# Xinglab/abPOA

Measured on AMD Instinct MI355X. Metric: read-sets/sec (consensus bit-exact) + DP Gcells/sec (roofline.dp_gcells_per_s), higher is better.
Workload: dtype int16

## Files before the change

abpoa_amd/csrc/engine.cpp:

```cpp
#include <hip/hip_runtime.h>
#include <stdio.h>
#include <stdlib.h>
#include <string.h>
#include <stdarg.h>
#include <limits.h>
#include <mutex>
#include <vector>
#include <algorithm>
#include "engine_options.h"
#include "batch_stream.h"
#include "dir_plane.h"

namespace abpoa_hip {

static char g_err[512] = ""; static std::mutex g_err_mu;
static thread_local char g_err_copy[512] = "";
static thread_local char tl_err[512] = "";
void set_err(const char *fmt, ...) {
    va_list ap; va_start(ap, fmt); vsnprintf(tl_err, sizeof(tl_err), fmt, ap); va_end(ap);
    std::lock_guard<std::mutex> lk(g_err_mu);
    memcpy(g_err, tl_err, sizeof(g_err));
}
const char *thread_last_error() { return tl_err; }
void clear_thread_error() { tl_err[0] = 0; }
// ... 184 lines not shown
                                b.lds.fr_cols > 0 &&
                                d.qlen <= b.lds.q_cap && !(dbg_ & 64);
            const bool dir_a = dir && fast_a && (dir_wide || !takes_wide_band(b.lds, d.w));
            d.plane_cap = dir_a ? (first_pass ? dir_est_cells_[todo[t]] : dir_full_cells_[todo[t]]) : (first_pass ? est_cells_[todo[t]] : full_cells_[todo[t]]);
            d.plane_off = plane_bytes; plane_bytes += (int64_t)align_up((size_t)d.plane_cap * (d.bits / 8) + 64 * 8 * 4);
            pass[t] = d;
        }
        if ((rc = planes_.reserve((size_t)plane_bytes))) return rc;
        memcpy(hi + o_desc_, pass.data(), sizeof(AlnDesc) * pass.size());
        b.o1 = sc->gap_open1; b.e1 = sc->gap_ext1; b.o2 = sc->gap_open2; b.e2 = sc->gap_ext2;
        b.align_mode = sc->align_mode; b.gap_mode = sc->gap_mode; b.wb = sc->wb; b.zdrop = sc->zdrop; b.ret_cigar = sc->ret_cigar; b.rev_cigar = sc->rev_cigar;
        b.want_trace = trace ? 1 : 0; b.fresh_band = fresh ? 1 : 0;
        b.dir_mode = dir ? (dir_wide ? 2 : 1) : 0; b.row_sdist = di + o_sdist_; b.row_pd = (const uint32_t *)(di + o_pd_);
        b.want_lr = (trace || (flags_ & BS_WANT_BAND_STATE)) ? 1 : 0;
        b.dbg = opt_int("ABPOA_HIP_DBG", 0);
        b.mat = (const int32_t *)(di + o_mat_); b.aln = (const AlnDesc *)(di + o_desc_); b.out = (AlnOut *)(dout + o_rec_);
        b.query = di + o_query_; b.row_base = di + o_base_; b.row_node_id = (const int32_t *)(di + o_nid_); b.row_remain = (const int32_t *)(di + o_rem_);
        b.row_active = di + o_act_; b.pred_off = (const int32_t *)(di + o_poff_); b.pred_row = (const int32_t *)(di + o_pred_);
        b.out_off = (const int32_t *)(di + o_ooff_); b.out_row = (const int32_t *)(di + o_out_);
        b.left = (int32_t *)(dout + o_left_); b.right = (int32_t *)(dout + o_right_);
        b.dp_beg_sn = (int32_t *)(dout + o_bsn_); b.dp_end_sn = (int32_t *)(dout + o_esn_); b.row_cell_off = (int64_t *)(dout + o_coff_);
        b.row_max_i = (int32_t *)(dout + o_rmi_); b.planes = planes_.dev; b.cigar = (uint64_t *)(dout + o_cig_);

        HIP_TRY(hipEventRecord(ev_[0], stream_), ABPOA_HIP_ELAUNCH);
        HIP_TRY(hipMemcpyAsync(di, hi, first_pass ? in_bytes_ : o_mat_, hipMemcpyHostToDevice, stream_), ABPOA_HIP_ELAUNCH);
        if (banded && !fresh) {
            if (first_pass) {
                saved_lr.assign((const int32_t *)(ho + o_left_), (const int32_t *)(ho + o_left_) + lr_words);
                HIP_TRY(hipMemcpyAsync(dout + o_left_, ho + o_left_, lr_words * 4, hipMemcpyHostToDevice, stream_), ABPOA_HIP_ELAUNCH);
            } else for (int i : todo) {
// ... 245 lines not shown
```

abpoa_amd/csrc/engine_options.cpp:

```cpp
#include "engine_options.h"
#include <atomic>
#include <cstdlib>
#include <cstring>
#include <mutex>
#include <string>

namespace abpoa_hip {
namespace {

struct Row { const char *name, *help; };
const Row kTable[] = {
    {"ABPOA_GPU_DEVICES", "P  device ordinals abpoa_hip_msa_batch spreads its batches over: all | 0,1,... (default: the device of abpoa_hip_init)"},
    {"ABPOA_GPU_BATCHES_PER_DEVICE", "P  batches dealt per device queue [2]"},
    {"ABPOA_HIP_STRICT", "P  1: a call that would hand any read-set to the host driver fails with ABPOA_HIP_ESTRICT"},
    {"ABPOA_HIP_VERBOSE", "P  per-pass timings, residency and fallback reasons on stderr"},
    {"ABPOA_HIP_HOSTGRAPH", "T  1: the host driver for every job"},
    {"ABPOA_HIP_NO_DEVICE_STRAND", "T  1: -s jobs on the host driver"},
    {"ABPOA_HIP_NO_DEVICE_LOCAL", "T  1: local-mode jobs on the host driver"},
    {"ABPOA_HIP_NO_DEVICE_GENERAL", "T  1: general-kernel jobs on the host driver"},
    {"ABPOA_HIP_DEVICE_GENERAL", "T  1: the general kernel for every device-resident job"},
    {"ABPOA_HIP_LOCKSTEP", "T  1: one launch per phase and round also where the all-rounds kernel would run"},
    {"ABPOA_HIP_LATE_TAIL", "T  1: the helpers of the all-rounds kernel's backtrack start after the row loop, not under it"},
    {"ABPOA_HIP_NODIR", "T  1: score-record arenas instead of direction words"},
    {"ABPOA_HIP_DIR_WIDE", "T  1 / 0: direction words for wide-band alignments always / never (default: by residency and memory)"},
    {"ABPOA_HIP_NOFAST", "T  1: no fast row loops (general kernel)"},
    {"ABPOA_HIP_NOWIDE", "T  1: no wide row loop"},
    {"ABPOA_HIP_NOXL", "T  1: no long-read form of the wide row loop"},
    {"ABPOA_HIP_LOCAL_TEAM", "T  1 / 0: the four-wavefront local row loop always / never"},
    {"ABPOA_HIP_WIDE_LO", "T  smallest band half-width that takes the wide loop [40]"},
    {"ABPOA_HIP_RING_ROWS", "T  depth of the wide loop's score ring (4 | 8 | 16)"},
    {"ABPOA_HIP_EXTRA_ROUTE_MIN", "T  ragged sets with fewer extra columns keep the narrow loop"},
    {"ABPOA_HIP_NO_RAGGED_SPLIT", "T  1: read-sets with ragged read ends stay in the batch of the uniform ones (no all-rounds kernel for such a job)"},
    {"ABPOA_HIP_RAGGED_CONCURRENT", "T  1: the ragged batch of a mixed job runs on a second queue of the device beside the uniform batch (measured: see LOG.md)"},
    {"ABPOA_HIP_PASS_SETS", "T  read-sets per pass of the device-resident driver"},
    {"ABPOA_HIP_FIRST_PASS", "T  start the node-slot ladder (3x, 4.5x, 6x, 4096x) at its second / third / fourth pass: 1 / 2 / 3 (profiling runs of one step)"},
    {"ABPOA_HIP_NO_PASS_HINT", "T  1: always start the ladder at 3x"},
    {"ABPOA_HIP_GROUPS", "T  read-set groups of the host driver"},
    {"ABPOA_HIP_ARENA_PCT", "T  arena estimate in percent (overflow-retry tests)"},
    {"ABPOA_HIP_BT_BYTES", "T  LDS window of the tail kernel in bytes"},
    {"ABPOA_HIP_BT_WC", "T  columns per row of the tail's column-slice windows"},
    {"ABPOA_HIP_ORDER_LDS", "T  0: the row-order walk with global tables"},
    {"ABPOA_HIP_ORDER_CAP", "T  node capacity of the row-order walk's LDS tables"},
    {"ABPOA_HIP_DBG", "D  bit mask handed to the kernels (DevBatch.dbg: 64 no fast loops, 128 keep counters, 1024 one wavefront per backtrack, 2048 the compiler's tight loop, ...)"},
    {"ABPOA_HIP_DEVSYNC", "D  1: compare device graph / row order / MSA with the host's after every read"},
    {"ABPOA_HIP_DEVICE_AUDIT", "D  1: every pool of a device queue must sit on that queue's device"},
    {"ABPOA_HIP_CIGAR_DIGEST", "D  1: fold every graph cigar into a per-set digest on the device"},
    {"ABPOA_HIP_DIRTRACE", "D  1: keep direction words and scores (word-level tests)"},
    {"ABPOA_HIP_IMBAL", "D  1: per-round mean / slowest alignment"},
    {"ABPOA_HIP_WIDE_COUNTERS", "D  path census of the wide loop (diagnostic build)"},
    {"ABPOA_HIP_ROW_CENSUS", "D  row census of the narrow loop (diagnostic build)"},
    {"ABPOA_HIP_ORDER_PROF", "D  in-kernel clock of the row-order walk (diagnostic build)"},
};
constexpr int N = (int)(sizeof(kTable) / sizeof(kTable[0]));

struct Snap { bool set[N]; std::string val[N]; };
std::mutex g_mu;
bool g_over_on[N]; std::string g_over[N];
std::atomic<const Snap *> g_snap{nullptr};
// ... 43 lines not shown
```

abpoa_amd/csrc/msa_device.cpp:

```cpp
#include <algorithm>
#include <atomic>
#include <chrono>
#include <limits.h>
#include <mutex>
#include <stdio.h>
#include <stdlib.h>
#include <string.h>
#include <thread>
#include <vector>
#include <hip/hip_runtime.h>
#include "engine_options.h"
#include "batch_stream.h"
#include "msa_device.h"
#include "poa_device.h"
#include "poa_graph.h"
#include "dir_plane.h"
#include "msa_batch.h"
#include "msa_device_debug.h"
#include "msa_device_plan.h"

namespace abpoa_hip {

namespace {
#define HIP_OK(expr, code) do { hipError_t e_ = (expr); if (e_ != hipSuccess) { \
// ... 283 lines not shown
    b.lds.narrow_off = (!mixed && b.lds.wide_on >= 1 && w_min >= b.lds.wide_w_lo && w_top <= b.lds.wide_w_hi) ? 1 : 0;
    return 0;
}

int fill_dev_batch(Job &J, bool *want_general) {
    const DevicePlan &pl = J.pl; Cache &C = *J.C; const Layout &L = J.L; const abpoa_hip_scoring_t *sc = &pl.sc; const PoaDev &p = J.p; DevBatch &b = J.b, &b_rc = J.b_rc;
    uint8_t *di = C.in.dev, *dr = C.rows.dev; const bool gen_io = pl.gen_io(); int rc;
    memset(&b, 0, sizeof(b));
    b.n = J.n_sets; b.m = sc->m;
    if ((rc = final_lds_plan(J, b))) return rc;
    if (!pl.local && !pl.general && (b.lds.fr_cols == 0 || pl.max_qlen > b.lds.q_cap)) { *want_general = true; set_err("band too wide for the fast row loop"); return ABPOA_HIP_EINVAL; }
    b.o1 = sc->gap_open1; b.e1 = sc->gap_ext1; b.o2 = sc->gap_open2; b.e2 = sc->gap_ext2;
    b.align_mode = sc->align_mode; b.gap_mode = sc->gap_mode; b.wb = sc->wb; b.zdrop = sc->zdrop; b.ret_cigar = 1; b.rev_cigar = 0;
    b.want_trace = 0; b.fresh_band = 1; b.want_lr = 0;
    b.dbg = opt_int("ABPOA_HIP_DBG", 0);
    b.mat = (const int32_t *)(di + L.o_mat); b.aln = p.aln; b.out = p.out;
    b.dir_mode = pl.dir ? (pl.dir_wide ? 2 : 1) : 0; b.row_sdist = p.row_sdist; b.row_pd = p.row_pd;
    b.query = p.reads; b.row_base = p.row_base; b.row_node_id = p.row_node_id; b.row_remain = p.row_remain; b.row_active = p.row_base;
    b.pred_off = p.pred_off; b.pred_row = p.pred_row; b.out_off = p.pred_off; b.out_row = p.pred_row;
    b.left = p.scratch; b.right = p.scratch;
    if (gen_io) {
        b.out_off = p.out_off; b.out_row = p.out_row; b.left = (int32_t *)(dr + L.o_left); b.right = (int32_t *)(dr + L.o_right); b.row_active = dr + L.o_act;
    }
    b.dp_beg_sn = (int32_t *)(dr + L.o_bsn); b.dp_end_sn = (int32_t *)(dr + L.o_esn); b.row_cell_off = (int64_t *)(dr + L.o_coff);
    b.row_max_i = (int32_t *)(dr + L.o_rmi);
    b.planes = C.planes.dev; b.cigar = p.cigar;
    b_rc = b;
    if (pl.amb) {
        b.want_lr = (sc->wb >= 0 && !pl.general) ? 1 : 0;
        b_rc = b; b_rc.want_lr = 0; b_rc.fresh_band = sc->wb >= 0 ? 0 : 1;
// ... 269 lines not shown
```

abpoa_amd/csrc/msa_device_debug.cpp:

```cpp
#include <algorithm>
#include <limits.h>
#include <stdio.h>
#include <stdlib.h>
#include <string.h>
#include "engine_options.h"
#include "msa_device_debug.h"

namespace abpoa_hip {

void consensus_flat(int n, const int32_t *order, const uint8_t *base, const uint8_t *nout, const int32_t *out_id, const int32_t *out_w,
                    const int32_t *n_read, std::vector<int> *ids, std::vector<uint8_t> *bases, std::vector<int> *cov, std::vector<int> &score,
                            std::vector<int> &max_out, int out_cap) {
    ids->clear(); bases->clear(); cov->clear();
    if (n <= 2) return;
    score.assign(n, 0); max_out.assign(n, -1);
    for (int r = n - 1; r >= 0; --r) {
        const int cur = order[r];
        const int32_t *oi = out_id + (size_t)cur * out_cap, *ow = out_w + (size_t)cur * out_cap; const int no = nout[cur];
        if (cur == 1) { max_out[cur] = -1; score[cur] = 0; }
        else if (cur == 0) {
            int path_score = -1, path_max_w = -1, max_id = -1;
            for (int i = 0; i < no; ++i) if (ow[i] > path_max_w || (ow[i] == path_max_w && score[oi[i]] > path_score)) { max_id = oi[i]; path_score =
                    score[oi[i]]; path_max_w = ow[i]; }
            max_out[cur] = max_id;
// ... 146 lines not shown
                                      "would take %.0f (int16 affine) -> rows keeping their records: ~%.1f %%\n", k, rd / n_sets, nc / n_sets,
                                      cu / n_sets / 16, nc / n_sets / 16, 100.0 * (cu - nc) / (4.0 * nc + 1)); }
    if (b.dbg & 128) {
        std::vector<std::pair<unsigned long long, int>> pl; for (int s_ = 0; s_ < n_sets; ++s_) { const unsigned long long h_ =
                (unsigned long long)ho[s_].seg[5]; pl.push_back({((h_ >> 32) & 15) << 16 | (h_ & 0xff30) , s_}); }
        std::sort(pl.begin(), pl.end()); double t_sh = 0, t_al = 0; int n_sh = 0, n_al = 0;
        for (size_t i_ = 0; i_ < pl.size(); ++i_) { const bool sh_ = (i_ > 0 && pl[i_ - 1].first == pl[i_].first) || (i_ + 1 < pl.size() && pl[i_
                + 1].first == pl[i_].first); (sh_ ? t_sh : t_al) += (double)ho[pl[i_].second].clk_dp; (sh_ ? n_sh : n_al)++; }
        fprintf(stderr, "[poa-device] round %d placement: %d alignments alone on their SIMD (mean ticks %.0f), %d sharing one (mean ticks %.0f)\n", k, n_al,
                n_al ? t_al / n_al : 0.0, n_sh, n_sh ? t_sh / n_sh : 0.0);
    }
    if ((b.dbg & 128) && opt_set("ABPOA_HIP_ROW_CENSUS")) {
        double rw[6] = {0, 0, 0, 0, 0, 0}, tk[6] = {0, 0, 0, 0, 0, 0}; for (const AlnOut &o_ : ho) for (int q_ = 0; q_ < 6; ++q_) {
                rw[q_] += (double)(o_.seg[q_] >> 40); tk[q_] += (double)(o_.seg[q_] & ((1ll << 40) - 1)); }
        const bool asmc_ = opt_int("ABPOA_HIP_ROW_CENSUS", 0) == 2;
        const char *nm_[5] = {asmc_ ? "assembly loop" : "1 predecessor", asmc_ ? "C++ 1-2 predecessors" : "2 predecessors", "3-8 predecessors (C++)", "all-chunks / exact bodies", "tile switches"};
        fprintf(stderr, "[poa-device] round %d narrow-loop census per alignment:", k);
        for (int q_ = 0; q_ < 5; ++q_) fprintf(stderr, " %s %.0f x %.0f ticks |", nm_[q_], rw[q_] / n_sets, rw[q_] > 0 ? tk[q_] / rw[q_] : 0.0);
        { int w_ = 0; for (int s_ = 0; s_ < n_sets; ++s_) if (ho[s_].clk_dp > ho[w_].clk_dp) w_ = s_; const AlnOut &o_ = ho[w_];
          fprintf(stderr, "\n[poa-device] round %d slowest row loop (set %d, %lld ticks):", k, w_, (long long)o_.clk_dp);
          for (int q_ = 0; q_ < 5; ++q_) fprintf(stderr, " %s %lld x %.0f |", nm_[q_], (long long)(o_.seg[q_] >> 40), (o_.seg[q_] >> 40)
                  ? (double)(o_.seg[q_] & ((1ll << 40) - 1)) / (double)(o_.seg[q_] >> 40) : 0.0);
          fprintf(stderr, " exact-body rows: > 4 predecessors %lld, straight-line declined %lld, beyond the ring %lld;", (long long)(o_.seg[5] >> 40),
                  (long long)((o_.seg[5] >> 20) & 0xfffff), (long long)(o_.seg[5] & 0xfffff)); }
        double why[3] = {0, 0, 0}; for (const AlnOut &o_ : ho) { why[0] += (double)(o_.seg[5] >> 40); why[1] += (double)((o_.seg[5] >> 20) & 0xfffff);
                why[2] += (double)(o_.seg[5] & 0xfffff); }
        fprintf(stderr, " exact-body rows: > 4 predecessors %.0f, straight-line body declined %.0f, predecessor beyond the ring %.0f\n", why[0] / n_sets,
                why[1] / n_sets, why[2] / n_sets);
    }
    if ((b.dbg & 128) && opt_set("ABPOA_HIP_WIDE_COUNTERS")) { int w_ = 0; for (int s_ = 0; s_ < n_sets; ++s_) if (ho[s_].clk_dp > ho[w_].clk_dp) w_ = s_;
            const AlnOut &o_ = ho[w_];
        fprintf(stderr,
                "[poa-device] round %d slowest row loop: set %d ticks %lld rows %d | all-chunk body %lld | not eligible "
                        "%lld | ring-geometry %lld | > 5 chunks %lld | slow vectors straddle %lld | key window / wrap %lld\n", k, w_, (long long)o_.clk_dp,
                        o_.n_rows_done, (long long)(o_.seg[0] & 0xffffffffll), (long long)o_.seg[1], (long long)o_.seg[2], (long long)o_.seg[3], (long long)o_.seg[4],
                        (long long)o_.seg[5]); }
    if (opt_set("ABPOA_HIP_WIDE_COUNTERS")) {
        double body = 0, xl32 = 0, xl16 = 0; for (const AlnOut &o_ : ho) { body += (double)(o_.seg[0] & 0xffffffffll); xl32 += (double)((o_.seg[0] >> 32) & 0xffff);
                xl16 += (double)(o_.seg[0] >> 48); }
        fprintf(stderr,
            "[poa-device] round %d wide-loop rows per alignment (diagnostic build): all-chunk body %.0f | not eligible "
                    "(preds > 8 / distance) %.0f | ring-geometry %.0f | > 5 chunks %.0f | slow vectors straddle %.0f | key " "window / wrap %.0f | "
                    "9-11-chunk bodies int32 %.0f int16 %.0f\n", k,
// ... 56 lines not shown
```

abpoa_amd/csrc/rows_fast.h:

```cpp
#pragma once
#include "dp_common.h"
#include "dir_plane.h"
#include "rows_tight_asm.h"
#include "wide_closed_forms.h"

namespace abpoa_hip {

template <typename T, int GAP> struct FastFmt { static constexpr int CW = GAP == 0 ? 2 : (GAP == 1 ? 4 : 8); };
static_assert(FastFmt<int, 0>::CW == record_values(ABPOA_HIP_LINEAR_GAP) && FastFmt<int, 1>::CW == record_values(ABPOA_HIP_AFFINE_GAP) && FastFmt<int, 2>::CW == record_values(ABPOA_HIP_CONVEX_GAP), "engine.h record_values");
template <typename T, int GAP> struct DirFmt {
    static constexpr int DB = GAP == 1 ? 2 : 4;
    static constexpr int UPV2 = Width<T>::PN * DB / 16;
    __device__ __host__ static constexpr int units(int nv) { return (nv * UPV2 + 1) >> 1; }
};
template <int GAP> __device__ __forceinline__ unsigned dir_word(unsigned kf, unsigned u1, unsigned u2, unsigned d1, unsigned d2) {
    static_assert(DIRA_DF1_SH - DIRA_UE1_SH == 3 && DIRC_UE2_SH - DIRC_UE1_SH == 3 && DIRC_DF2_SH - DIRC_DF1_SH == 3 && DIRC_DF1_SH - DIRC_UE1_SH == 8, "field layout of dir_plane.h");
    if (GAP == 1) return (((d1 << 3) | u1) << DIRA_UE1_SH) | kf;
    return (((((d2 << 3) | d1) << 8) | ((u2 << 3) | u1)) << DIRC_UE1_SH) | kf;
}
template <int GAP> __device__ __forceinline__ unsigned dir_pack(unsigned kM, unsigned kE1, unsigned kE2, unsigned u1, unsigned u2, unsigned d1, unsigned d2) {
    return dir_word<GAP>(GAP == 1 ? (kE1 << DIRA_KE1_SH) | kM : (((kE2 << 4) | kE1) << DIRC_KE1_SH) | kM, u1, u2, d1, d2);
}
__device__ __forceinline__ unsigned umin_(unsigned a, unsigned b) { return a < b ? a : b; }
template <typename T> __device__ __forceinline__ unsigned dir_literal(int Hm1, int Fm1, int F, int oe, int e) {
// ... 111 lines not shown
    const int fast_lo = (int)lo_ll;
    const int kconst = I16 ? argmax_key16_const(PN, l, vvl) : 0;
    const int ktie = argmax_tie32(PN, l, vvl);

    { GLOBAL_AS const int32_t *g_mat = vgpr_ptr(b.mat); for (int i = lane; i < m * m1; i += 64) { const int bb = i / m1, qc = i - bb * m1; s_mx[i] = qc < m ? g_mat[bb * m + qc] : 0; } }
    for (int i = lane; i < RR * NPW * RCS; i += 64) { const int pl = (i / RCS) % NPW; fr[i] = (I16 && pl == 0) ? infw : ((EPACK && pl == 1) ? 0 : inf); }
    WG_SYNC();
    auto ring_put = [&](int slot, int x, int H, int E1, int E2) __attribute__((always_inline)) {
        int *q = fr + slot * (NPW * RCS) + 2 + x;
        if (I16) { q[0] = (int)(((unsigned)H & 0xffffu) | ((unsigned)E1 << 16)); if (GAP == 2) q[RCS] = E2; }
        else { q[0] = H; if (GAP != 0) q[RCS] = E1; if (GAP == 2) q[2 * RCS] = E2; }
    };

    const bool extend = sgpr(b.align_mode == ABPOA_HIP_EXTEND_MODE ? 1 : 0) != 0;
    int ex_best = inf, ex_i = 0, ex_j = 0, ex_rem = 0; bool zstop = false;
    const bool asm_tight_on = sgpr(!(b.dbg & 2048) && RC == 128 && b.align_mode != ABPOA_HIP_EXTEND_MODE ? 1 : 0) != 0;
    int cur = 0, n_vec_lane = 0;
    const int cap_pn = (int)(d.plane_cap / PN > 0x7fffffffLL ? 0x7fffffffLL : d.plane_cap / PN);
    const int cap_turbo = cap_pn - (DIR ? dir_units(NV) + NV * CWR : NV * CW);
    const int remain_end = __builtin_amdgcn_readfirstlane(io.row_remain[gn - 1]);
    int vg_geo = 0, vg_mi = 0, vg_off = 0;
    int vg_vm = 0, rowmax = 0;
    {
        const int r = __builtin_amdgcn_readfirstlane(io.row_remain[0]) - remain_end - 1;
        const int dp_end0 = imin(qlen, imax(0, qlen - r) + w);
        const int end_sn0 = dp_end0 / PN, W0 = (end_sn0 + 1) * PN;
        if ((long long)W0 * CWR > d.plane_cap) { status = ABPOA_HIP_STATUS_OVERFLOW; cursor_out = 0; n_cells_out = 0; rows_done_out = 0; return; }
        const bool ring0 = W0 <= RC && !EPACK;
        T *H = io.planes;
        for (int i = lane; i < W0; i += 64) {
// ... 543 lines not shown
            const unsigned kb = (unsigned)__builtin_amdgcn_readlane((int)akey, 63);
            rowmax = (int)(kb >> 16) - 32768;
            mi = (rowmax > inf) ? beg_sn * PN + (int)(kb & 63) : -1;
        } else {
            const int vmax = __builtin_amdgcn_readlane(aval, 63);
            rowmax = vmax;
            const unsigned key = (am_ok && hsE_ == vmax) ? (((unsigned)(PN - 1 - l) << 12) | (unsigned)((vvl == nvr - 1) ? 8 : NV - 1 - vvl)) : 0u;
            const unsigned kb = wave_max_u32_s(key);
            const int vrel = (kb & 8) ? nvr - 1 : NV - 1 - (int)(kb & 7);
            mi = (vmax > inf) ? (beg_sn + vrel) * PN + (PN - 1 - (int)((kb >> 12) & 0xf)) : -1;
        }
        return 1;
    };
    auto turbo_body = [&](auto npc, auto slowc, int row, int ti) __attribute__((always_inline)) -> int {
        if constexpr (GAP == 0) return turbo_lin(npc, slowc, row, ti); else return turbo_aff(npc, slowc, row, ti);
    };

    constexpr int NCHX = XL ? 11 : 7;
    int two_chunk_streak = 0;
    int qcx_beg_sn = -1, qoffx[NCHX] = {};
    int ilp_far = 0;
    auto ilp_band = [&](int row, int ti) __attribute__((always_inline)) -> int {
        int mn_mi, mx_mi, min_pb;
        ilp_far = 0;
        auto is_far = [&](int p, int g_) __attribute__((always_inline)) { return (row - p >= RR || !(g_ & GEO_RING)) ? 1 : 0; };
        {
            const int p = __builtin_amdgcn_readlane(tv_p0, ti), g_ = __builtin_amdgcn_readlane(vg_geo, p & 63);
            mn_mi = mx_mi = __builtin_amdgcn_readlane(vg_mi, p & 63); min_pb = g_ & 0xfff; max_pe = (g_ >> 12) & 0xfff; ilp_far = is_far(p, g_);
        }
        auto more = [&](int tvp, int k) __attribute__((always_inline)) {
// ... 372 lines not shown
                if (mx > ex_best) { ex_best = mx; ex_i = t0 + ti; ex_j = mi; ex_rem = rem_row; }
                else if (b.zdrop > 0) { int dd = (ex_rem - rem_row) - (mi - ex_j); if (dd < 0) dd = -dd; if (ex_best - mx > b.zdrop + e1 * dd) zstop = true; }
            }
            if constexpr (WIDEB || !I16) {
                const int vm_new = sgpr(rowmax);
                asm volatile("s_mov_b32 m0, %8\n\ts_nop 3\n\tv_writelane_b32 %0, %4, m0\n\tv_writelane_b32 %1, %5, m0\n\tv_writelane_b32 %2, %6, m0\n\tv_writelane_b32 %3, %7, m0"
                             : "+v"(vg_geo), "+v"(vg_mi), "+v"(vg_off), "+v"(vg_vm) : "s"(geo_new), "s"(mi), "s"(off_new), "s"(vm_new), "s"(ti) : "m0");
            } else
            asm volatile("s_mov_b32 m0, %6\n\ts_nop 3\n\tv_writelane_b32 %0, %3, m0\n\tv_writelane_b32 %1, %4, m0\n\tv_writelane_b32 %2, %5, m0"
                         : "+v"(vg_geo), "+v"(vg_mi), "+v"(vg_off) : "s"(geo_new), "s"(mi), "s"(off_new), "s"(ti) : "m0");
        };
        int row = imax(t0, 1);
        while (row < r_hi && !zstop) {
            int ok_ = 1;
            if constexpr (!WIDEB && GAP != 0) if (__builtin_expect(two_chunk_streak, 0)) {
                const int ti_ = row & 63, meta_ = __builtin_amdgcn_readlane(tv_meta, ti_);
                if constexpr (DIR) row_spill = (meta_ >> 21) & 1;
                if ((meta_ >> 19) & 1) {
                    CENSUS_T0()
                    last_done = row;
                    rterm = __builtin_amdgcn_readlane(tv_rterm, ti_); base = meta_ & 0xff; np = (meta_ >> 8) & 0xff;
                    const int nch_ = ilp_band(row, ti_);
                    if (nch_ == -2) { status = ABPOA_HIP_STATUS_OVERFLOW; break; }
                    if (nch_ == 2 && ilp_chunks(std::integral_constant<int, 2>{}, nch_, row, ti_) == 1) { commit_row(ti_, true); CENSUS(3) ++row; continue; }
                }
                two_chunk_streak = 0;
            }
            bool cxx_tight = true;
#if !defined(ABPOA_HIP_ABLATE) && !defined(ABPOA_HIP_PROFILE) && (!defined(ABPOA_HIP_ROW_CENSUS) || defined(ABPOA_HIP_ASM_CENSUS)) && !defined(ABPOA_HIP_NO_ASM_TIGHT)
            if constexpr (!WIDEB && I16 && GAP == 1 && DIR) {
                if (asm_tight_on && cur + NV * (r_hi - row) <= cap_turbo) {
                    int code, sM, sTB, sRT, sR2, sP0, sM0, sG0, sSL0, sA, sB, sESN, sBSN, sPB0, sPE0, sNV1, sC0, sP1, sM1, sG1, sSL1, sPB1, sPE1, sP2, sSL2, sPB2, sPE2, sP3, sSL3, sPB3, sPE3;
                    long long inb, amok, msk;
#ifdef ABPOA_HIP_ASM_CENSUS
                    const int asm_row0 = row; const long long asm_t0 = (long long)__builtin_amdgcn_s_memtime();
#endif
                    int infw_v = infw, inf_v = inf; asm("" : "+v"(infw_v), "+v"(inf_v));
                    const int mxb = (int)(unsigned)(size_t)(lds_int_t *)s_mx, qb = (int)(unsigned)(size_t)(lds_int_t *)(const void *)s_query;
                    asm volatile(TIGHT_ASM_I16_AFFINE_DIR
                        : [row] "+s"(row), [cur] "+s"(cur), [qcb] "+s"(qc_beg_sn), [code] "=&s"(code), [geo] "+v"(vg_geo), [mi] "+v"(vg_mi), [off] "+v"(vg_off), [qoff0] "+v"(qoff0),
                          [qoff1] "+v"(qoff1), [sM] "=&s"(sM), [sTB] "=&s"(sTB), [sRT] "=&s"(sRT), [sR2] "=&s"(sR2), [sP0] "=&s"(sP0), [sM0] "=&s"(sM0), [sG0] "=&s"(sG0), [sSL0] "=&s"(sSL0), [sA] "=&s"(sA),
// ... 37 lines not shown
            base = meta & 0xff; np = (meta >> 8) & 0xff;
            if constexpr (DIR) row_spill = (meta >> 21) & 1;
            if (!WIDEB && ((meta >> 18) & 1)) {
                if (turbo_body(std::integral_constant<int, 4>{}, std::true_type{}, row, ti) == 1) { commit_row(ti, true); CENSUS(2) ++row; continue; }
            }
            if (!WIDEB && ((meta >> 20) & 1)) {
                if (turbo_body(std::integral_constant<int, 8>{}, std::true_type{}, row, ti) == 1) { commit_row(ti, true); CENSUS(2) ++row; continue; }
            }
            if (!WIDEB && (((meta >> 17) & 1) ? ok_ == 0 : (DIR && ((meta >> 22) & 1)))) {
                const int ok3 = np == 1 ? turbo_body(std::integral_constant<int, 1>{}, std::true_type{}, row, ti) : turbo_body(std::integral_constant<int, 2>{}, std::true_type{}, row, ti);
                if (ok3 == 1) { commit_row(ti, true); CENSUS(np == 1 ? 0 : 1) ++row; continue; }
            }
            if (GAP != 0 && !WIDEB && ((meta >> 19) & 1)) {
                const int nch_ = ilp_band(row, ti);
                if (nch_ == -2) { status = ABPOA_HIP_STATUS_OVERFLOW; break; }
                if (nch_ >= 1 && nch_ <= 2 && ilp_chunks(std::integral_constant<int, 2>{}, nch_, row, ti) == 1) { two_chunk_streak = nch_ == 2; commit_row(ti, true); CENSUS(3) ++row; continue; }
            }
            if (WIDEB && ((meta >> 19) & 1)) {
                const int nch_ = ilp_band(row, ti);
                if (nch_ == -2) { status = ABPOA_HIP_STATUS_OVERFLOW; break; }
                if (nch_ >= 2) {
                    int ok2;
                    if (nch_ <= 3) ok2 = ilp_chunks(std::integral_constant<int, 3>{}, nch_, row, ti);
                    else if (nch_ == 4) ok2 = ilp_chunks(std::integral_constant<int, 4>{}, nch_, row, ti);
                    else if (nch_ == 5) ok2 = ilp_chunks(std::integral_constant<int, 5>{}, nch_, row, ti);
                    else if (nch_ == 6) ok2 = ilp_chunks(std::integral_constant<int, 6>{}, nch_, row, ti);
                    else if (nch_ <= 7) ok2 = ilp_chunks(std::integral_constant<int, 7>{}, nch_, row, ti);
                    else if constexpr (XL) {
                        if (nch_ == 8) ok2 = ilp_chunks(std::integral_constant<int, 8>{}, nch_, row, ti);
                        else if (nch_ == 9) ok2 = ilp_chunks(std::integral_constant<int, 9>{}, nch_, row, ti);
                        else ok2 = ilp_chunks(std::integral_constant<int, 11>{}, nch_, row, ti);
// ... 20 lines not shown
                } else {
                    const int vmax = wave_max_i32_s(am_any ? am_val : INT_MIN);
                    rowmax = vmax;
                    if (vmax > inf) {
                        unsigned key = 0;
                        if (am_any && am_val == vmax) key = ((unsigned)(PN - 1 - l) << 27) | ((unsigned)am_isend << 26) | (0x3FFFFFFu - (unsigned)am_v);
                        const unsigned kb = wave_max_u32_s(key);
                        mi = (int)(0x3FFFFFFu - (kb & 0x3FFFFFFu)) * PN + (PN - 1 - (int)(kb >> 27));
                        if (mi > qlen) mi = -1;
                    }
                }
            }
            commit_row(ti, to_ring);
            FSTAMP(4)
            CENSUS(3)
#ifdef ABPOA_HIP_ROW_CENSUS
            fseg[5] += np > 4 ? (1ll << 40) : (((meta >> 16) & 1) ? (1ll << 20) : 1ll);
#endif
            ++row;
        }
        if (status != 0) break;
    }
    if (status == 0) {
        const int tb = last_done & ~63, rb = tb + lane;
        if (rb <= last_done) { io.g_bsn[rb] = vg_geo & 0xfff; io.g_esn[rb] = (vg_geo >> 12) & 0xfff; io.g_coff[rb] = (long long)(uint32_t)vg_off * PN; io.row_max_i[rb] = vg_mi;
                               if (rb >= 1) n_vec_lane += ((vg_geo >> 12) & 0xfff) - (vg_geo & 0xfff) + 1; }
    }
    WG_SYNC();
    if (status == 0 && b.want_lr) {
        const int push_lim = zstop ? last_done : gn;
        for (int r = lane; r < gn; r += 64) {
            int lf = gn, rt = 0;
            if (r == 0) { lf = 0; rt = 0; }
// ... 52 lines not shown
```

Baseline: 19570.

## Add lean two-chunk row body for streaks of two-chunk rows in narrow loop

Adds a specialized turbo_aff2 body that computes affine-gap DP rows spanning exactly two 64-lane chunks. It merges up to four predecessors, runs the DPP prefix scan and writes the ring, plane and direction words in one unrolled pass. Once a two-chunk row succeeds in the narrow loop, following rows run this lean body in a tight inner loop instead of re-entering the general ilp_band/ilp_chunks dispatch. The aim is to cut per-row dispatch and generic chunk overhead. It adds a large new code path that must stay bit-exact, with fallbacks to the general path when band or wrap checks fail, plus an env/dbg switch to disable it.

```diff
diff --git a/abpoa_amd/csrc/engine.cpp b/abpoa_amd/csrc/engine.cpp
--- a/abpoa_amd/csrc/engine.cpp
+++ b/abpoa_amd/csrc/engine.cpp
@@ -222,6 +222,7 @@
         b.dir_mode = dir ? (dir_wide ? 2 : 1) : 0; b.row_sdist = di + o_sdist_; b.row_pd = (const uint32_t *)(di + o_pd_);
         b.want_lr = (trace || (flags_ & BS_WANT_BAND_STATE)) ? 1 : 0;
         b.dbg = opt_int("ABPOA_HIP_DBG", 0);
+        if (opt_set("ABPOA_HIP_TWO_CHUNK_LEAN") && !opt_on("ABPOA_HIP_TWO_CHUNK_LEAN")) b.dbg |= 4096;
         b.mat = (const int32_t *)(di + o_mat_); b.aln = (const AlnDesc *)(di + o_desc_); b.out = (AlnOut *)(dout + o_rec_);
         b.query = di + o_query_; b.row_base = di + o_base_; b.row_node_id = (const int32_t *)(di + o_nid_); b.row_remain = (const int32_t *)(di + o_rem_);
         b.row_active = di + o_act_; b.pred_off = (const int32_t *)(di + o_poff_); b.pred_row = (const int32_t *)(di + o_pred_);
diff --git a/abpoa_amd/csrc/engine_options.cpp b/abpoa_amd/csrc/engine_options.cpp
--- a/abpoa_amd/csrc/engine_options.cpp
+++ b/abpoa_amd/csrc/engine_options.cpp
@@ -25,6 +25,7 @@
     {"ABPOA_HIP_DIR_WIDE", "T  1 / 0: direction words for wide-band alignments always / never (default: by residency and memory)"},
     {"ABPOA_HIP_NOFAST", "T  1: no fast row loops (general kernel)"},
     {"ABPOA_HIP_NOWIDE", "T  1: no wide row loop"},
+    {"ABPOA_HIP_TWO_CHUNK_LEAN", "T  0: rows of two chunks in the narrow row loop take the all-chunks body from the dispatch chain, one by one (default 1: streaks of them run the lean two-chunk body, rows_fast.h turbo_aff2)"},
     {"ABPOA_HIP_NOXL", "T  1: no long-read form of the wide row loop"},
     {"ABPOA_HIP_LOCAL_TEAM", "T  1 / 0: the four-wavefront local row loop always / never"},
     {"ABPOA_HIP_WIDE_LO", "T  smallest band half-width that takes the wide loop [40]"},
@@ -41,7 +42,7 @@
     {"ABPOA_HIP_BT_WC", "T  columns per row of the tail's column-slice windows"},
     {"ABPOA_HIP_ORDER_LDS", "T  0: the row-order walk with global tables"},
     {"ABPOA_HIP_ORDER_CAP", "T  node capacity of the row-order walk's LDS tables"},
-    {"ABPOA_HIP_DBG", "D  bit mask handed to the kernels (DevBatch.dbg: 64 no fast loops, 128 keep counters, 1024 one wavefront per backtrack, 2048 the compiler's tight loop, ...)"},
+    {"ABPOA_HIP_DBG", "D  bit mask handed to the kernels (DevBatch.dbg: 64 no fast loops, 128 keep counters, 1024 one wavefront per backtrack, 2048 the compiler's tight loop, 4096 no lean two-chunk body, ...)"},
     {"ABPOA_HIP_DEVSYNC", "D  1: compare device graph / row order / MSA with the host's after every read"},
     {"ABPOA_HIP_DEVICE_AUDIT", "D  1: every pool of a device queue must sit on that queue's device"},
     {"ABPOA_HIP_CIGAR_DIGEST", "D  1: fold every graph cigar into a per-set digest on the device"},
diff --git a/abpoa_amd/csrc/msa_device.cpp b/abpoa_amd/csrc/msa_device.cpp
--- a/abpoa_amd/csrc/msa_device.cpp
+++ b/abpoa_amd/csrc/msa_device.cpp
@@ -321,6 +321,7 @@
     b.align_mode = sc->align_mode; b.gap_mode = sc->gap_mode; b.wb = sc->wb; b.zdrop = sc->zdrop; b.ret_cigar = 1; b.rev_cigar = 0;
     b.want_trace = 0; b.fresh_band = 1; b.want_lr = 0;
     b.dbg = opt_int("ABPOA_HIP_DBG", 0);
+    if (opt_set("ABPOA_HIP_TWO_CHUNK_LEAN") && !opt_on("ABPOA_HIP_TWO_CHUNK_LEAN")) b.dbg |= 4096;
     b.mat = (const int32_t *)(di + L.o_mat); b.aln = p.aln; b.out = p.out;
     b.dir_mode = pl.dir ? (pl.dir_wide ? 2 : 1) : 0; b.row_sdist = p.row_sdist; b.row_pd = p.row_pd;
     b.query = p.reads; b.row_base = p.row_base; b.row_node_id = p.row_node_id; b.row_remain = p.row_remain; b.row_active = p.row_base;
diff --git a/abpoa_amd/csrc/msa_device_debug.cpp b/abpoa_amd/csrc/msa_device_debug.cpp
--- a/abpoa_amd/csrc/msa_device_debug.cpp
+++ b/abpoa_amd/csrc/msa_device_debug.cpp
@@ -184,19 +184,15 @@
         double rw[6] = {0, 0, 0, 0, 0, 0}, tk[6] = {0, 0, 0, 0, 0, 0}; for (const AlnOut &o_ : ho) for (int q_ = 0; q_ < 6; ++q_) {
                 rw[q_] += (double)(o_.seg[q_] >> 40); tk[q_] += (double)(o_.seg[q_] & ((1ll << 40) - 1)); }
         const bool asmc_ = opt_int("ABPOA_HIP_ROW_CENSUS", 0) == 2;
-        const char *nm_[5] = {asmc_ ? "assembly loop" : "1 predecessor", asmc_ ? "C++ 1-2 predecessors" : "2 predecessors", "3-8 predecessors (C++)", "all-chunks / exact bodies", "tile switches"};
+        const char *nm_[6] = {asmc_ ? "assembly loop" : "1 predecessor", asmc_ ? "C++ 1-2 predecessors" : "2 predecessors", "3-8 predecessors (C++)", "all-chunks / exact bodies", "tile switches",
+                              "lean two-chunk body"};
         fprintf(stderr, "[poa-device] round %d narrow-loop census per alignment:", k);
-        for (int q_ = 0; q_ < 5; ++q_) fprintf(stderr, " %s %.0f x %.0f ticks |", nm_[q_], rw[q_] / n_sets, rw[q_] > 0 ? tk[q_] / rw[q_] : 0.0);
+        for (int q_ = 0; q_ < 6; ++q_) fprintf(stderr, " %s %.0f x %.0f ticks |", nm_[q_], rw[q_] / n_sets, rw[q_] > 0 ? tk[q_] / rw[q_] : 0.0);
         { int w_ = 0; for (int s_ = 0; s_ < n_sets; ++s_) if (ho[s_].clk_dp > ho[w_].clk_dp) w_ = s_; const AlnOut &o_ = ho[w_];
           fprintf(stderr, "\n[poa-device] round %d slowest row loop (set %d, %lld ticks):", k, w_, (long long)o_.clk_dp);
-          for (int q_ = 0; q_ < 5; ++q_) fprintf(stderr, " %s %lld x %.0f |", nm_[q_], (long long)(o_.seg[q_] >> 40), (o_.seg[q_] >> 40)
+          for (int q_ = 0; q_ < 6; ++q_) fprintf(stderr, " %s %lld x %.0f |", nm_[q_], (long long)(o_.seg[q_] >> 40), (o_.seg[q_] >> 40)
                   ? (double)(o_.seg[q_] & ((1ll << 40) - 1)) / (double)(o_.seg[q_] >> 40) : 0.0);
-          fprintf(stderr, " exact-body rows: > 4 predecessors %lld, straight-line declined %lld, beyond the ring %lld;", (long long)(o_.seg[5] >> 40),
-                  (long long)((o_.seg[5] >> 20) & 0xfffff), (long long)(o_.seg[5] & 0xfffff)); }
-        double why[3] = {0, 0, 0}; for (const AlnOut &o_ : ho) { why[0] += (double)(o_.seg[5] >> 40); why[1] += (double)((o_.seg[5] >> 20) & 0xfffff);
-                why[2] += (double)(o_.seg[5] & 0xfffff); }
-        fprintf(stderr, " exact-body rows: > 4 predecessors %.0f, straight-line body declined %.0f, predecessor beyond the ring %.0f\n", why[0] / n_sets,
-                why[1] / n_sets, why[2] / n_sets);
+          fprintf(stderr, "\n"); }
     }
     if ((b.dbg & 128) && opt_set("ABPOA_HIP_WIDE_COUNTERS")) { int w_ = 0; for (int s_ = 0; s_ < n_sets; ++s_) if (ho[s_].clk_dp > ho[w_].clk_dp) w_ = s_;
             const AlnOut &o_ = ho[w_];
diff --git a/abpoa_amd/csrc/rows_fast.h b/abpoa_amd/csrc/rows_fast.h
--- a/abpoa_amd/csrc/rows_fast.h
+++ b/abpoa_amd/csrc/rows_fast.h
@@ -149,6 +149,7 @@
 
     const bool extend = sgpr(b.align_mode == ABPOA_HIP_EXTEND_MODE ? 1 : 0) != 0;
     int ex_best = inf, ex_i = 0, ex_j = 0, ex_rem = 0; bool zstop = false;
+    const bool lean2_on = sgpr(!(b.dbg & 4096) ? 1 : 0) != 0;
     const bool asm_tight_on = sgpr(!(b.dbg & 2048) && RC == 128 && b.align_mode != ABPOA_HIP_EXTEND_MODE ? 1 : 0) != 0;
     int cur = 0, n_vec_lane = 0;
     const int cap_pn = (int)(d.plane_cap / PN > 0x7fffffffLL ? 0x7fffffffLL : d.plane_cap / PN);
@@ -722,6 +723,203 @@
     };
     auto turbo_body = [&](auto npc, auto slowc, int row, int ti) __attribute__((always_inline)) -> int {
         if constexpr (GAP == 0) return turbo_lin(npc, slowc, row, ti); else return turbo_aff(npc, slowc, row, ti);
+    };
+    auto turbo_aff2 = [&](int row, int ti) __attribute__((always_inline)) -> int {
+        const int tb = __builtin_amdgcn_readlane(tv_tb, ti);
+        const int p0 = row - (tb & 0xff);
+        const int g0 = __builtin_amdgcn_readlane(vg_geo, p0 & 63), m0 = __builtin_amdgcn_readlane(vg_mi, p0 & 63);
+        int mn = m0, mx = m0, min_pb = g0 & 0xfff, ring = g0; max_pe = (g0 >> 12) & 0xfff;
+        int p1 = p0, g1 = g0, p2 = p0, g2 = g0, p3 = p0, g3 = g0;
+        if (np > 1) {
+            p1 = row - ((tb >> 8) & 0xff);
+            g1 = __builtin_amdgcn_readlane(vg_geo, p1 & 63); const int m1_ = __builtin_amdgcn_readlane(vg_mi, p1 & 63);
+            mn = imin(mn, m1_); mx = imax(mx, m1_); min_pb = imin(min_pb, g1 & 0xfff); max_pe = imax(max_pe, (g1 >> 12) & 0xfff); ring &= g1;
+            if (np > 2) {
+                p2 = __builtin_amdgcn_readlane(tv_p2, ti); p3 = np > 3 ? __builtin_amdgcn_readlane(tv_p3, ti) : p2;
+                g2 = __builtin_amdgcn_readlane(vg_geo, p2 & 63); g3 = __builtin_amdgcn_readlane(vg_geo, p3 & 63);
+                const int m2_ = __builtin_amdgcn_readlane(vg_mi, p2 & 63), m3_ = __builtin_amdgcn_readlane(vg_mi, p3 & 63);
+                mn = imin(mn, imin(m2_, m3_)); mx = imax(mx, imax(m2_, m3_));
+                min_pb = imin(min_pb, imin(g2 & 0xfff, g3 & 0xfff)); max_pe = imax(max_pe, imax((g2 >> 12) & 0xfff, (g3 >> 12) & 0xfff)); ring &= g2 & g3;
+            }
+        }
+        mn = sgpr(mn); mx = sgpr(mx);
+        set_band(std::true_type{}, mn, mx, min_pb);
+        const int nvr = end_sn - beg_sn + 1, Wr = nvr * PN, relv_end = end_sn - beg_sn;
+        const int okbits = (NV - nvr) & (nvr - 2 * NV - 1) & (Wr - RC - 1) & (beg_sn - max_pe - 1) & (cur + row_units(nvr, row_spill) - cap_pn - 1) & (ring << 7);
+        if (__builtin_expect(okbits >= 0, 0)) return 0;
+        if (end_sn > max_pe && (max_pe + 1 - beg_sn) / NV != 1) return 0;
+        if (__builtin_expect(beg_sn != qc_beg_sn, 0)) {
+            qc_beg_sn = beg_sn;
+            const int c0 = beg_sn * PN + lane, c1 = c0 + 64;
+            qoff0 = (c0 >= 1 && c0 <= qlen) ? qat(c0 - 1) : m; qoff1 = (c1 >= 1 && c1 <= qlen) ? qat(c1 - 1) : m;
+        }
+        const int colb = beg_sn * PN + lane;
+        int q[2];
+        q[0] = *(const int *)((const char *)s_mx + (tb >> 16) + qoff0 * 4); q[1] = *(const int *)((const char *)s_mx + (tb >> 16) + qoff1 * 4);
+        auto ring_read2 = [&](int p, int g_, int c, int &r0, int &r1, int &r2) __attribute__((always_inline)) {
+            const int x = colb + 64 * c - (g_ & 0xfff) * PN;
+            const int *src = ring_at(__builtin_amdgcn_readlane(vslot, p), med3i(x - 1, -2, RC));
+            r2 = inf;
+            if (I16) { r0 = src[0]; r1 = src[1]; if (GAP == 2) r2 = src[RCS + 1]; }
+            else { r0 = src[0]; r1 = src[RCS + 1]; if (GAP == 2) r2 = src[2 * RCS + 1]; }
+        };
+        int Mv[2], E1v[2], E2v[2], kb[2], kE1[2], kE2[2];
+        auto merge2 = [&](int g_, int c, int r0, int r1, int r2, int kidx) __attribute__((always_inline)) {
+            int hm1, ev1, ev2 = inf;
+            if (I16) { hm1 = (int)(short)r0; ev1 = r1 >> 16; ev2 = r2; } else { hm1 = r0; ev1 = r1; ev2 = r2; }
+            const int pb = g_ & 0xfff, Wp = (((g_ >> 12) & 0xfff) - pb + 1) * PN, x = colb + 64 * c - pb * PN;
+            const bool inH = (unsigned)x < (unsigned)(Wp + PN), inE = (unsigned)x < (unsigned)Wp;
+            kb[c] = (inH && hm1 > Mv[c]) ? kidx : kb[c];
+            if (DIR) { kE1[c] = (inE && ev1 > E1v[c]) ? kidx : kE1[c]; if (GAP == 2) kE2[c] = (inE && ev2 > E2v[c]) ? kidx : kE2[c]; }
+            Mv[c] = inH ? imax(Mv[c], hm1) : Mv[c]; E1v[c] = inE ? imax(E1v[c], ev1) : E1v[c]; if (GAP == 2) E2v[c] = inE ? imax(E2v[c], ev2) : E2v[c];
+        };
+        {
+            int ra0[2], ra1[2], ra2[2], rb0[2] = {0, 0}, rb1[2] = {0, 0}, rb2[2] = {inf, inf};
+#pragma unroll
+            for (int c = 0; c < 2; ++c) ring_read2(p0, g0, c, ra0[c], ra1[c], ra2[c]);
+            if (np > 1) {
+#pragma unroll
+                for (int c = 0; c < 2; ++c) ring_read2(p1, g1, c, rb0[c], rb1[c], rb2[c]);
+            }
+#pragma unroll
+            for (int c = 0; c < 2; ++c) {
+                if (I16) { Mv[c] = (int)(short)ra0[c]; E1v[c] = ra1[c] >> 16; E2v[c] = ra2[c]; } else { Mv[c] = ra0[c]; E1v[c] = ra1[c]; E2v[c] = ra2[c]; }
+                kb[c] = 1; kE1[c] = 1; kE2[c] = 1;
+            }
+            if (np > 1) {
+#pragma unroll
+                for (int c = 0; c < 2; ++c) merge2(g1, c, rb0[c], rb1[c], rb2[c], 2);
+                if (np > 2) {
+                    int rc0[2], rc1[2], rc2[2], rd0[2], rd1[2], rd2[2];
+#pragma unroll
+                    for (int c = 0; c < 2; ++c) { ring_read2(p2, g2, c, rc0[c], rc1[c], rc2[c]); ring_read2(p3, g3, c, rd0[c], rd1[c], rd2[c]); }
+#pragma unroll
+                    for (int c = 0; c < 2; ++c) { merge2(g2, c, rc0[c], rc1[c], rc2[c], 3); merge2(g3, c, rd0[c], rd1[c], rd2[c], 4); }
+                }
+            }
+        }
+        int h[2], hs[2], hsE[2], lowest = INT_MAX;
+#pragma unroll
+        for (int c = 0; c < 2; ++c) {
+            h[c] = wr(Mv[c] + q[c]);
+            hs[c] = h[c]; if (GAP == 2) hs[c] = imax(imax(h[c], E1v[c]), E2v[c]);
+            hsE[c] = GAP == 1 ? imax(h[c], E1v[c]) : hs[c];
+            lowest = imin(lowest, h[c]);
+        }
+        const bool wrap_here = __any(lowest < fast_lo);
+        if (__builtin_expect(wrap_here, 0)) return 0;
+        int g1s[2], g2s[2], s1[2], s2[2];
+#pragma unroll
+        for (int c = 0; c < 2; ++c) { g1s[c] = hs[c] + le1; s1[c] = wave_shr1(INT_MIN, g1s[c]); if (GAP == 2) { g2s[c] = hs[c] + le2; s2[c] = wave_shr1(INT_MIN, g2s[c]); } }
+        const bool in_band1 = 64 + lane < Wr, is_end1 = NV + vvl == relv_end;
+        const int vfloor = I16 ? 0 : __builtin_amdgcn_readlane(vg_vm, p0 & 63) - (1 << 19);
+        unsigned amk;
+        {
+            int cand1 = hsE[1]; if (end_sn == qlen_sn) cand1 = (is_end1 && colb + 64 > qlen) ? inf : cand1;
+            unsigned k0, k1;
+            if (I16) { k0 = argmax_key16(hsE[0], kconst, beg_sn, false); k1 = argmax_key16(cand1, kconst, beg_sn + NV, is_end1); }
+            else { k0 = argmax_key32(hsE[0], vfloor, ktie, 0, NV, false); k1 = argmax_key32(cand1, vfloor, ktie, 1, NV, is_end1); }
+            amk = (in_band1 && k1 > k0) ? k1 : k0;
+        }
+        {
+            auto step = [&](auto ctrl, auto rmask) __attribute__((always_inline)) {
+                constexpr int CT = decltype(ctrl)::value, RM = decltype(rmask)::value;
+#pragma unroll
+                for (int c = 0; c < 2; ++c) {
+                    s1[c] = imax(s1[c], __builtin_amdgcn_update_dpp(INT_MIN, s1[c], CT, RM, 0xF, false));
+                    if (GAP == 2) s2[c] = imax(s2[c], __builtin_amdgcn_update_dpp(INT_MIN, s2[c], CT, RM, 0xF, false));
+                }
+                const unsigned t = (unsigned)__builtin_amdgcn_update_dpp(0, (int)amk, CT, RM, 0xF, false); amk = t > amk ? t : amk;
+            };
+            step(std::integral_constant<int, 0x111>{}, std::integral_constant<int, 0xF>{});
+            step(std::integral_constant<int, 0x112>{}, std::integral_constant<int, 0xF>{});
+            step(std::integral_constant<int, 0x114>{}, std::integral_constant<int, 0xF>{});
+            step(std::integral_constant<int, 0x118>{}, std::integral_constant<int, 0xF>{});
+            step(std::integral_constant<int, 0x142>{}, std::integral_constant<int, 0xA>{});
+            step(std::integral_constant<int, 0x143>{}, std::integral_constant<int, 0xC>{});
+        }
+        const unsigned kbst = (unsigned)__builtin_amdgcn_readlane((int)amk, 63);
+        int seed1[2], seed2[2];
+        seed1[0] = __builtin_amdgcn_readlane(h[0], 0) - e1; seed2[0] = seed1[0] + e1 - e2;
+        asm("" : "+v"(seed1[0])); if (GAP == 2) asm("" : "+v"(seed2[0]));
+        seed1[1] = carry_next(__builtin_amdgcn_readlane(imax(s1[0], g1s[0]), 63), seed1[0], e1);
+        if (GAP == 2) seed2[1] = carry_next(__builtin_amdgcn_readlane(imax(s2[0], g2s[0]), 63), seed2[0], e2); else seed2[1] = INT_MIN;
+        if (!I16) { if (__builtin_expect(argmax_declines32(kbst), 0)) return 0; }
+        T *const Hrow = io.planes + (long long)cur * PN + (long long)lane * CWR;
+        off_pn = cur + ((DIR && row_spill) ? nvr * CWR : 0); cur += row_units(nvr, row_spill);
+        char *const Drow = (char *)io.planes + (size_t)off_pn * 32 + (size_t)lane * DB;
+        int *const qd = (int *)ring_at(__builtin_amdgcn_readlane(vslot, ti) + 4 * lane, 0);
+        int F1[2], F2[2], S1[2], S2[2];
+#pragma unroll
+        for (int c = 0; c < 2; ++c) {
+            S1[c] = imax(s1[c], seed1[c]); F1[c] = imax(S1[c] - cf1, inj1); F2[c] = inf; S2[c] = 0;
+            if (GAP == 2) { S2[c] = imax(s2[c], seed2[c]); F2[c] = imax(S2[c] - cf2, inj2); }
+        }
+        const bool lit = end_sn > max_pe;
+        if (__builtin_expect(lit, 0)) {
+            const int vb = beg_sn + NV;
+            const int nvec = imin(NV, end_sn - vb + 1), nfast = imax(0, imin(nvec, max_pe - vb + 1));
+            int first, first2 = 0;
+            if (nfast > 0) {
+                const int lastl = nfast * PN - 1;
+                first = __builtin_amdgcn_readlane(imax(S1[1], g1s[1]), lastl) - lastl * e1;
+                if (GAP == 2) first2 = __builtin_amdgcn_readlane(imax(S2[1], g2s[1]), lastl) - lastl * e2;
+            } else { first = __builtin_amdgcn_readfirstlane(seed1[1]) + e1; if (GAP == 2) first2 = __builtin_amdgcn_readfirstlane(seed2[1]) + e2; }
+            T f1t = (T)F1[1], f2t = (T)F2[1], fi = (T)first, fi2 = (T)first2;
+            slow_f_vectors<T, GAP>(vb, end_sn, max_pe, nfast, l, vvl, (T)hs[1], (T)inf, (T)e1, (T)oe1, (T)o1, (T)e2, (T)oe2, (T)o2, f1t, f2t, fi, fi2);
+            F1[1] = (int)f1t; F2[1] = (int)f2t;
+        }
+#pragma unroll
+        for (int c = 0; c < 2; ++c) {
+            const bool in_band = c == 0 ? true : in_band1;
+            int Hout, E1out, E2out = inf, t2a, t2b = 0, en_a = 0;
+            if (GAP == 1) {
+                Hout = imax(hsE[c], F1[c]);
+                t2a = wr(Hout - oe1); if (DIR) asm("" : "+v"(t2a));
+                en_a = imax(wr(E1v[c] - e1), t2a);
+                E1out = (Hout == hsE[c]) ? en_a : inf;
+            } else {
+                Hout = imax(hs[c], imax(F1[c], F2[c]));
+                t2a = wr(Hout - oe1); t2b = wr(Hout - oe2); if (DIR) asm("" : "+v"(t2a), "+v"(t2b));
+                E1out = imax(wr(E1v[c] - e1), t2a);
+                E2out = imax(wr(E2v[c] - e2), t2b);
+            }
+            const int mflag = (Mv[c] + q[c] == Hout) ? kb[c] : 0;
+            const int he = (int)(((unsigned)Hout & 0xffffu) | ((unsigned)E1out << 16));
+            if constexpr (DIR) {
+                const unsigned u1 = (unsigned)((GAP == 1 ? en_a : E1out) - t2a), d1 = umin_((unsigned)(Hout - F1[c]), (unsigned)CAPF1);
+                unsigned u2 = 0, d2 = 0;
+                if (GAP == 2) { u2 = (unsigned)(E2out - t2b); d2 = umin_((unsigned)(Hout - F2[c]), (unsigned)CAPF2); }
+                unsigned wd = dir_pack<GAP>((unsigned)mflag, (unsigned)kE1[c], (unsigned)kE2[c], u1, u2, d1, d2);
+                if (c == 1) if (__builtin_expect(lit, 0)) {
+                    const int vb = beg_sn + NV, nfast_ = imax(0, imin(imin(NV, end_sn - vb + 1), max_pe - vb + 1));
+                    const int Hp_ = GAP == 1 ? imax(hsE[0], F1[0]) : imax(hs[0], imax(F1[0], F2[0]));
+                    const int pH = __builtin_amdgcn_readlane(Hp_, 63), pF1 = __builtin_amdgcn_readlane(F1[0], 63), pF2 = __builtin_amdgcn_readlane(F2[0], 63);
+                    const int Hm1 = wave_shr1(pH, Hout), F1m1 = wave_shr1(pF1, F1[c]);
+                    unsigned l1 = dir_literal<T>(Hm1, F1m1, F1[c], oe1, e1), l2 = 0;
+                    if (GAP == 2) { const int F2m1 = wave_shr1(pF2, F2[c]); l2 = dir_literal<T>(Hm1, F2m1, F2[c], oe2, e2); }
+                    if (vvl >= nfast_) wd |= GAP == 1 ? l1 << DIRA_LF1_SH : (l1 << DIRC_LF1_SH | l2 << DIRC_LF2_SH);
+                }
+                char *const dp = Drow + c * 64 * DB;
+                if (GAP == 1) *(uint16_t *)dp = (uint16_t)wd; else *(uint32_t *)dp = wd;
+            }
+            if (DIR && !row_spill) {}
+            else if (DIR && !in_band) {}
+            else {
+                T *H = Hrow + c * 64 * CWR;
+                if (I16 && GAP == 1) { int2 rec; rec.x = he; rec.y = (int)__builtin_amdgcn_perm((unsigned)mflag, (unsigned)F1[c], 0x05040100u); *(int2 *)H = rec; }
+                else if (I16) { int4 rec; rec.x = he; rec.y = (int)(((unsigned)E2out & 0xffffu) | ((unsigned)F1[c] << 16)); rec.z = F2[c] & 0xffff; rec.w = mflag; *(int4 *)H = rec; }
+                else if (GAP == 1) { int4 rec; rec.x = Hout; rec.y = E1out; rec.z = F1[c]; rec.w = mflag; *(int4 *)H = rec; }
+                else { int4 r0, r1; r0.x = Hout; r0.y = E1out; r0.z = E2out; r0.w = F1[c]; r1.x = F2[c]; r1.y = mflag; r1.z = 0; r1.w = 0; ((int4 *)H)[0] = r0; ((int4 *)H)[1] = r1; }
+            }
+            if (I16) { qd[c * 64] = in_band ? he : infw; if (GAP == 2) qd[RCS + c * 64] = in_band ? E2out : inf; }
+            else { qd[c * 64] = in_band ? Hout : inf; qd[RCS + c * 64] = in_band ? E1out : inf; if (GAP == 2) qd[2 * RCS + c * 64] = in_band ? E2out : inf; }
+        }
+        for (int c = 2; c < (RC >> 6); ++c) { qd[c * 64] = infw; if (NPW > 1) qd[RCS + c * 64] = inf; if (NPW > 2) qd[2 * RCS + c * 64] = inf; }
+        mi = -1;
+        if (I16) { rowmax = argmax_value16(kbst); if (rowmax > inf) mi = argmax_index16(kbst, PN, qlen); }
+        else { rowmax = argmax_value32(kbst, vfloor); if (rowmax > inf) mi = argmax_index32(kbst, PN, beg_sn, qlen); }
+        return 1;
     };
 
     constexpr int NCHX = XL ? 11 : 7;
@@ -1124,17 +1322,18 @@
         while (row < r_hi && !zstop) {
             int ok_ = 1;
             if constexpr (!WIDEB && GAP != 0) if (__builtin_expect(two_chunk_streak, 0)) {
-                const int ti_ = row & 63, meta_ = __builtin_amdgcn_readlane(tv_meta, ti_);
-                if constexpr (DIR) row_spill = (meta_ >> 21) & 1;
-                if ((meta_ >> 19) & 1) {
+                for (;;) {
+                    const int ti_ = row & 63, meta_ = __builtin_amdgcn_readlane(tv_meta, ti_);
+                    if (!((meta_ >> 16) & 1)) { two_chunk_streak = 0; break; }
+                    if constexpr (DIR) row_spill = (meta_ >> 21) & 1;
                     CENSUS_T0()
-                    last_done = row;
                     rterm = __builtin_amdgcn_readlane(tv_rterm, ti_); base = meta_ & 0xff; np = (meta_ >> 8) & 0xff;
-                    const int nch_ = ilp_band(row, ti_);
-                    if (nch_ == -2) { status = ABPOA_HIP_STATUS_OVERFLOW; break; }
-                    if (nch_ == 2 && ilp_chunks(std::integral_constant<int, 2>{}, nch_, row, ti_) == 1) { commit_row(ti_, true); CENSUS(3) ++row; continue; }
+                    if (turbo_aff2(row, ti_) != 1) { two_chunk_streak = 0; break; }
+                    commit_row(ti_, true);
+                    CENSUS(5)
+                    if (++row >= r_hi || zstop) break;
                 }
-                two_chunk_streak = 0;
+                if (row >= r_hi || zstop) { last_done = row - 1; break; }
             }
             bool cxx_tight = true;
 #if !defined(ABPOA_HIP_ABLATE) && !defined(ABPOA_HIP_PROFILE) && (!defined(ABPOA_HIP_ROW_CENSUS) || defined(ABPOA_HIP_ASM_CENSUS)) && !defined(ABPOA_HIP_NO_ASM_TIGHT)
@@ -1202,7 +1401,7 @@
             if (GAP != 0 && !WIDEB && ((meta >> 19) & 1)) {
                 const int nch_ = ilp_band(row, ti);
                 if (nch_ == -2) { status = ABPOA_HIP_STATUS_OVERFLOW; break; }
-                if (nch_ >= 1 && nch_ <= 2 && ilp_chunks(std::integral_constant<int, 2>{}, nch_, row, ti) == 1) { two_chunk_streak = nch_ == 2; commit_row(ti, true); CENSUS(3) ++row; continue; }
+                if (nch_ >= 1 && nch_ <= 2 && ilp_chunks(std::integral_constant<int, 2>{}, nch_, row, ti) == 1) { two_chunk_streak = nch_ == 2 && lean2_on; commit_row(ti, true); CENSUS(3) ++row; continue; }
             }
             if (WIDEB && ((meta >> 19) & 1)) {
                 const int nch_ = ilp_band(row, ti);
@@ -1253,9 +1452,6 @@
             commit_row(ti, to_ring);
             FSTAMP(4)
             CENSUS(3)
-#ifdef ABPOA_HIP_ROW_CENSUS
-            fseg[5] += np > 4 ? (1ll << 40) : (((meta >> 16) & 1) ? (1ll << 20) : 1ll);
-#endif
             ++row;
         }
         if (status != 0) break;
```

New measurement: 19710 (median of 3 runs). About the same (+0.7%).
